# rwl/blu

Hardware: AMD Instinct MI355X
Metric: factorize nnz/s + achieved HBM GB/s, 100k x 100k 10-nnz/col basis (higher is better)
Workload: dtype f64

## Files before the change

### blu_amd/csrc/k_chain.h

```cpp
#pragma once
#include "blu_dev.h"

#define CH_SB 32
#define CH_NB 8
#define CH_CS (CH_SB * CH_NB)
#define CH_CE 4096
#define CH_W 2048
#define CH_FAR 320
#define CH_HAS 0x10000
#define CH_HT 16
#define CH_SEL_FAR (-1)
#define CH_SEL_PREV (-2)
#define CH_R 4
#define CH_TG 64
#define CH_SPIN 64

struct __attribute__((aligned(16))) ChRecA {
    int n, eb, w, k;
};
struct __attribute__((aligned(16))) ChRecB {
    double diag, own;
};
struct __attribute__((aligned(16))) ChOpsV {
    double val, xv;
};
struct ChainLds {
    ChOpsV ev[CH_CE];
    int sel[CH_CE];
    double xwin[CH_W];
    ChRecA ra[CH_CS];
    ChRecB rb[CH_CS];
    double rinit[CH_CS];
    long long s_b[CH_CS];
    volatile int blk_ready[CH_NB];
    volatile int eb_tag[CH_HT];
    volatile int eb_val[CH_HT];
    volatile int tag[CH_TG];
    volatile int ring_done[CH_R];
    volatile int ring_eb[CH_R];
    volatile int abort;
};

struct ChMeta {
    long long b;
    int len;
    int w;
    double diag, own;
};
struct ChEnt {
    int pos;
    int gidx;
    double val;
};

#ifdef BLU_EMU_BUILD
#define CH_LDS(T) T *
#else
#define CH_LDS(T) __attribute__((address_space(3))) T *
#endif
__device__ __forceinline__ int ch_flag(const volatile int *p) { return *(CH_LDS(const volatile int))p; }
__device__ __forceinline__ void ch_set(volatile int *p, int v) { *(CH_LDS(volatile int))p = v; }

#define CH_WAIT_SPIN(L, cond, code, spin, gave_up)                  \
    do {                                                            \
        int it_ = 0;                                                \
        while (!(cond)) {                                           \
            if (++it_ <= (spin)) continue;                          \
            if (ch_flag(&(L)->abort) || it_ > (1 << 24)) {                    \
                if (!ch_flag(&(L)->abort)) ch_set(&(L)->abort, (code));               \
                (gave_up) = true;                                   \
                break;                                              \
            }                                                       \
            __builtin_amdgcn_s_sleep(1);                            \
        }                                                           \
    } while (0)
#define CH_WAIT(L, cond, code)                       \
    do {                                             \
        bool gu_ = false;                            \
        CH_WAIT_SPIN(L, cond, code, 0, gu_);         \
    } while (0)

#ifdef BLU_EMU_BUILD
__device__ __forceinline__ void ch_lds_fence() {}
__device__ __forceinline__ void ch_vm_drain() {}
#else
__device__ __forceinline__ void ch_lds_fence() { asm volatile("s_waitcnt lgkmcnt(0)" ::: "memory"); }
__device__ __forceinline__ void ch_vm_drain() { asm volatile("s_waitcnt vmcnt(0)" ::: "memory"); }
#endif
__device__ __forceinline__ double ch_load_final(gdouble_p p)
{
    const long long b = __hip_atomic_load((GPTR(const long long))p, __ATOMIC_RELAXED, __HIP_MEMORY_SCOPE_AGENT);
    return __longlong_as_double(b);
}

__device__ __forceinline__ bool ch_room(ChainLds *L, int b, int top)
{
    int done = ch_flag(&L->ring_done[0]), eb = ch_flag(&L->ring_eb[0]);
#pragma unroll
    for (int r = 1; r < CH_R; r++) {
        const int d = ch_flag(&L->ring_done[r]), e = ch_flag(&L->ring_eb[r]);
        done = d < done ? d : done;
        eb = e < eb ? e : eb;
    }
    return done >= b - CH_NB + 1 && top - eb <= CH_CE;
}
template <bool INIT_OWN, bool SUB, class A>
__device__ __forceinline__ void ch_stage_block(const A &ad, ChainLds *L, int b, int k0, int dir, int nsteps, gdouble_p out)
{
    const int lane = lane_id();
    const int s0 = b * CH_SB;
    const int ns = nsteps - s0 < CH_SB ? nsteps - s0 : CH_SB;
    const int k = k0 + dir * (s0 + (lane < ns ? lane : 0));
    ChMeta M = ad.meta(k);
    if (M.len < 0) M.len = 0;
    const bool mine = lane < ns;
    const int st = (mine && M.len <= 64) ? M.len : 0;
    const int incl = wave_incl_scan_i(st);
    const int off = incl - st;
    const int cnt = __builtin_amdgcn_readlane(incl, 63);
    int base = 0;
    if (b > 0) {
        CH_WAIT(L, ch_flag(&L->eb_tag[b & (CH_HT - 1)]) == b, 1);
        base = ch_flag(&L->eb_val[b & (CH_HT - 1)]);
    }
    if (lane == 0) {
        ch_set(&L->eb_val[(b + 1) & (CH_HT - 1)], base + cnt);
        ch_lds_fence();
        ch_set(&L->eb_tag[(b + 1) & (CH_HT - 1)], b + 1);
    }
    CH_WAIT(L, ch_room(L, b, base + cnt), 2);
    asm volatile("" ::: "memory");
    if (ch_flag(&L->abort)) return;
    const int slot0 = s0 & (CH_CS - 1);
    if (mine) {
        const int sl = slot0 + lane;
        ChRecA a;
        a.n = M.len <= 64 ? (M.len > 0 ? (M.len | CH_HAS) : 0) : -1;
        a.eb = base + off;
        a.w = M.w;
        a.k = k;
        L->ra[sl] = a;
        ChRecB bq;
        bq.diag = M.diag;
        bq.own = M.own;
        L->rb[sl] = bq;
        L->rinit[sl] = INIT_OWN ? M.own : 0.0;
        L->s_b[sl] = M.b;
    }
    ch_lds_fence();
    for (int f0 = 0; f0 < cnt; f0 += 256) {
        int tt[4], ee[4];
        ChEnt E[4];
        bool ok[4], far[4];
        double xo[4];
#pragma unroll
        for (int u = 0; u < 4; u++) {
            const int f = f0 + u * 64 + lane;
            ok[u] = f < cnt;
            int lo = 0, hi = ns - 1;
            const int target = base + (ok[u] ? f : 0);
#pragma unroll
            for (int it = 0; it < 5; it++) {
                const int mid = (lo + hi + 1) >> 1;
                const bool ge = (L->ra[slot0 + mid].eb <= target) && (mid <= hi);
                lo = ge ? mid : lo;
                hi = ge ? hi : mid - 1;
            }
            tt[u] = lo;
            ee[u] = target - L->ra[slot0 + lo].eb;
        }
#pragma unroll
        for (int u = 0; u < 4; u++) {
            E[u].pos = 0;
            E[u].gidx = 0;
            E[u].val = 0.0;
            if (ok[u]) E[u] = ad.ent(L->ra[slot0 + tt[u]].k, L->s_b[slot0 + tt[u]], ee[u]);
        }
#pragma unroll
        for (int u = 0; u < 4; u++) {
            const int kk = L->ra[slot0 + tt[u]].k;
            const int d = (kk - E[u].pos) * dir;
            far[u] = ok[u] && d >= CH_FAR;
            xo[u] = 0.0;
            if (far[u]) xo[u] = ch_load_final(out + E[u].gidx);
        }
#pragma unroll
        for (int u = 0; u < 4; u++) {
            if (ok[u]) {
                const int kk = L->ra[slot0 + tt[u]].k;
                const int r = (base + f0 + u * 64 + lane) & (CH_CE - 1);
                ChOpsV ov;
                ov.val = E[u].val;
                ov.xv = xo[u];
                L->ev[r] = ov;
                L->sel[r] = far[u] ? CH_SEL_FAR : (E[u].pos == kk - dir ? CH_SEL_PREV : (E[u].pos & (CH_W - 1)));
            }
        }
    }
    ch_lds_fence();
    if (mine && M.len > 0 && M.len <= 64) {
        const int sl = slot0 + lane;
        const int eb = base + off;
        double acc = INIT_OWN ? M.own : 0.0;
        int p = 0;
        while (p < M.len && L->sel[(eb + p) & (CH_CE - 1)] == CH_SEL_FAR) {
            const ChOpsV ov = L->ev[(eb + p) & (CH_CE - 1)];
            const double term = __dmul_rn(ov.xv, ov.val);
            acc = SUB ? __dsub_rn(acc, term) : __dadd_rn(acc, term);
            p++;
        }
        if (p > 0) {
            L->ra[sl].n = (M.len - p) | CH_HAS;
            L->ra[sl].eb = eb + p;
            L->rinit[sl] = acc;
        }
    }
    ch_lds_fence();
    if (lane == 0) ch_set(&L->blk_ready[b & (CH_NB - 1)], b + 1);
}

struct ChRec {
    int n, eb, w, k;
    double diag, own, init;
};
struct ChOps {
    double val, xv;
    int sel;
};
__device__ __forceinline__ ChRec ch_read_rec(ChainLds *L, int s)
{
    const int sl = s & (CH_CS - 1);
    const ChRecA a = L->ra[sl];
    const ChRecB b = L->rb[sl];
    ChRec R;
    R.n = a.n;
    R.eb = a.eb;
    R.w = a.w;
    R.k = a.k;
    R.diag = b.diag;
    R.own = b.own;
    R.init = L->rinit[sl];
    return R;
}
template <bool SUB>
__device__ __forceinline__ double ch_accumulate(double acc, double prod, int n)
{
    const unsigned lo = (unsigned)__double_as_longlong(prod), hi = (unsigned)(__double_as_longlong(prod) >> 32);
#define CH_TERM(T)                                                                                              \
    {                                                                                                           \
        const unsigned a_ = __builtin_amdgcn_readlane(lo, (T)), b_ = __builtin_amdgcn_readlane(hi, (T));        \
        const double term_ = __longlong_as_double((long long)(((unsigned long long)b_ << 32) | a_));            \
        acc = SUB ? __dsub_rn(acc, term_) : __dadd_rn(acc, term_);                                              \
    }
    int t = 0;
    for (; t + 4 <= n; t += 4) {
        CH_TERM(t)
        CH_TERM(t + 1)
        CH_TERM(t + 2)
        CH_TERM(t + 3)
    }
    for (; t < n; t++) CH_TERM(t)
#undef CH_TERM
    return acc;
}

template <bool SUB>
__device__ __forceinline__ double ch_accumulate_rows(double acc, double prod, int n)
{
    const double sg = SUB ? -1.0 : 1.0;
#ifdef BLU_EMU_BUILD
#define CH_D(T) acc = fma(__shfl(prod, (lane_id() & ~15) + T), sg, acc);
#define CH_D0 CH_D(0)
#else
#define CH_D(T) asm volatile("v_fmac_f64_dpp %0, %1, %2 row_newbcast:" #T " row_mask:0xf bank_mask:0xf" : "+v"(acc) : "v"(prod), "v"(sg));
#define CH_D0 asm volatile("s_nop 4\n\tv_fmac_f64_dpp %0, %1, %2 row_newbcast:0 row_mask:0xf bank_mask:0xf" : "+v"(acc) : "v"(prod), "v"(sg));
#endif
#define CH_TAIL(A, B, C) \
    if (n > A) {         \
        CH_D(A)          \
        if (n > B) {     \
            CH_D(B)      \
            if (n > C) { \
                CH_D(C)  \
            }            \
        }                \
    }
    if (n >= 4) {
        CH_D0 CH_D(1) CH_D(2) CH_D(3)
        if (n >= 8) {
            CH_D(4) CH_D(5) CH_D(6) CH_D(7)
            if (n >= 12) {
                CH_D(8) CH_D(9) CH_D(10) CH_D(11)
                if (n >= 16) {
                    CH_D(12) CH_D(13) CH_D(14) CH_D(15)
                } else {
                    CH_TAIL(12, 13, 14)
                }
            } else {
                CH_TAIL(8, 9, 10)
            }
        } else {
            CH_TAIL(4, 5, 6)
        }
    } else if (n > 0) {
        CH_D0
        CH_TAIL(1, 2, 3)
    }
#undef CH_TAIL
#undef CH_D0
#undef CH_D
    return acc;
}

template <bool INIT_OWN, bool SUB, class A, class F>
__device__ __forceinline__ bool chain_sweep(const A &ad, ChainLds *L, int k0, int dir, int nsteps, gdouble_p out, F f)
{
    static_assert(CH_R >= 1 && CH_R <= CH_SB && CH_TG >= 2 * CH_R, "ring size");
    const int w = wave_id(), nw = num_waves(), lane = lane_id();
    const int nblk = (nsteps + CH_SB - 1) / CH_SB;
    if (threadIdx.x < CH_NB) ch_set(&L->blk_ready[threadIdx.x], 0);
    if (threadIdx.x < CH_HT) ch_set(&L->eb_tag[threadIdx.x], -1);
    if (threadIdx.x < CH_TG) ch_set(&L->tag[threadIdx.x], 0);
    if (threadIdx.x < CH_R) {
        ch_set(&L->ring_done[threadIdx.x], 0);
        ch_set(&L->ring_eb[threadIdx.x], 0);
    }
    if (threadIdx.x == 0) ch_set(&L->abort, 0);
    __syncthreads();
    if (w >= CH_R) {
        for (int b = w - CH_R; b < nblk && !ch_flag(&L->abort); b += nw - CH_R) ch_stage_block<INIT_OWN, SUB>(ad, L, b, k0, dir, nsteps, out);
    } else {
#ifdef BLU_PROFILE
        long long t_wait = 0, t_tag = 0, t_drain = 0;
        const long long t_begin = (long long)__builtin_amdgcn_s_memtime();
#endif
        const int last = nsteps - 1;
        const int li = lane & 15;
        __builtin_amdgcn_s_setprio(3);
        const auto rl_d = [](double x, int t) {
            const int lo = __builtin_amdgcn_readlane(__double2loint(x), t), hi = __builtin_amdgcn_readlane(__double2hiint(x), t);
            return __hiloint2double(hi, lo);
        };
        const auto read_ops = [&](int eb, int n) {
            ChOps E;
            E.val = 0.0;
            E.xv = 0.0;
            E.sel = CH_SEL_FAR;
            const int l = n <= 16 ? li : lane;
            if (l < n) {
                const int r = (eb + l) & (CH_CE - 1);
                const ChOpsV v = L->ev[r];
                E.val = v.val;
                E.xv = v.xv;
                E.sel = L->sel[r];
            }
            return E;
        };
        int cur_b = -1;
        ChRec BR;
        BR.n = BR.eb = BR.w = BR.k = 0;
        BR.diag = BR.own = BR.init = 0.0;
        bool gave_up = false;
        for (int s = w; s < nsteps && !gave_up; s += CH_R) {
            const int b = s / CH_SB;
            if (b != cur_b) {
                if (cur_b >= 0) {
#ifdef BLU_PROFILE
                    const long long td0 = (long long)__builtin_amdgcn_s_memtime();
#endif
                    ch_vm_drain();
#ifdef BLU_PROFILE
                    t_drain += (long long)__builtin_amdgcn_s_memtime() - td0;
#endif
                    ch_lds_fence();
                    if (lane == 0) ch_set(&L->ring_done[w], b);
                }
#ifdef BLU_PROFILE
                const long long tw0 = (long long)__builtin_amdgcn_s_memtime();
#endif
                CH_WAIT_SPIN(L, ch_flag(&L->blk_ready[b & (CH_NB - 1)]) == b + 1, 3, 0, gave_up);
                asm volatile("" ::: "memory");
#ifdef BLU_PROFILE
                t_wait += (long long)__builtin_amdgcn_s_memtime() - tw0;
#endif
                if (gave_up) break;
                const int sl = b * CH_SB + lane;
                BR = ch_read_rec(L, sl < last ? sl : last);
                if (lane == 0) ch_set(&L->ring_eb[w], BR.eb);
                cur_b = b;
            }
            const int t = s - b * CH_SB;
            const int nf = __builtin_amdgcn_readlane(BR.n, t), eb1 = __builtin_amdgcn_readlane(BR.eb, t);
            const int k1 = __builtin_amdgcn_readlane(BR.k, t), w1 = __builtin_amdgcn_readlane(BR.w, t);
            const double own1 = rl_d(BR.own, t), diag1 = rl_d(BR.diag, t);
            const int n1 = nf < 0 ? -1 : (nf & (CH_HAS - 1));
            double acc = rl_d(BR.init, t);
            const auto wait_prev = [&]() {
                if (s > 0) {
#ifdef BLU_PROFILE
                    const long long tw0 = (long long)__builtin_amdgcn_s_memtime();
#endif
                    CH_WAIT_SPIN(L, ch_flag(&L->tag[(s - 1) & (CH_TG - 1)]) == s, 4, CH_SPIN, gave_up);
#ifdef BLU_PROFILE
                    t_tag += (long long)__builtin_amdgcn_s_memtime() - tw0;
#endif
                }
                asm volatile("" ::: "memory");
            };
            const auto slot_of = [&](int sel) { return (sel == CH_SEL_PREV ? k1 - dir : sel) & (CH_W - 1); };
            const auto dist_of = [&](int slot) { return ((k1 - slot) * dir) & (CH_W - 1); };
            if (n1 > 0 && n1 <= 16) {
                const ChOps E = read_ops(eb1, n1);
                const int slot = slot_of(E.sel);
                const bool win = E.sel != CH_SEL_FAR;
                const bool late = win && dist_of(slot) < CH_R;
                const unsigned lm = (unsigned)__ballot(late) & 0xffffu;
                const int p = lm ? __ffs((int)lm) - 1 : n1;
                if (p > 0) {
                    const double x = (win && !late) ? L->xwin[slot] : E.xv;
                    acc = ch_accumulate_rows<SUB>(acc, li < p ? __dmul_rn(x, E.val) : 0.0, p);
                }
                if (p < n1) {
                    const int nl = n1 - p;
                    const ChOps EL = read_ops(eb1 + p, nl);
                    const int slot_l = slot_of(EL.sel);
                    const bool win_l = EL.sel != CH_SEL_FAR;
                    const bool late_l = win_l && dist_of(slot_l) < CH_R;
                    const double prod_e = __dmul_rn((win_l && !late_l) ? L->xwin[slot_l] : EL.xv, EL.val);
                    wait_prev();
                    const double prod_l = __dmul_rn(L->xwin[slot_l], EL.val);
                    acc = ch_accumulate_rows<SUB>(acc, li < nl ? (late_l ? prod_l : prod_e) : 0.0, nl);
                } else {
                    wait_prev();
                }
            } else if (n1 > 16) {
                const ChOps E = read_ops(eb1, n1);
                wait_prev();
                const double x = E.sel != CH_SEL_FAR ? L->xwin[slot_of(E.sel)] : E.xv;
                acc = ch_accumulate<SUB>(acc, lane < n1 ? __dmul_rn(x, E.val) : 0.0, n1);
            } else if (n1 < 0) {
                wait_prev();
                const ChMeta M = ad.meta(k1);
                for (int o = 0; o < M.len; o += 64) {
                    ChEnt E;
                    E.pos = k1 - dir * CH_FAR;
                    E.gidx = 0;
                    E.val = 0.0;
                    const int nn = M.len - o < 64 ? M.len - o : 64;
                    double x = 0.0;
                    if (lane < nn) {
                        E = ad.ent(k1, M.b, o + lane);
                        const int d = (k1 - E.pos) * dir;
                        x = (d > 0 && d < CH_FAR) ? L->xwin[E.pos & (CH_W - 1)] : ch_load_final(out + E.gidx);
                    }
                    acc = ch_accumulate<SUB>(acc, lane < nn ? __dmul_rn(x, E.val) : 0.0, nn);
                }
            } else {
                wait_prev();
            }
            if (gave_up) break;
            const double v = f(k1, nf != 0, acc, own1, diag1);
            if (lane == 0) {
                L->xwin[k1 & (CH_W - 1)] = v;
                ch_lds_fence();
                ch_set(&L->tag[s & (CH_TG - 1)], s + 1);
                out[w1] = v;
            }
        }
        __builtin_amdgcn_s_setprio(0);
        ch_vm_drain();
        ch_lds_fence();
        if (lane == 0) {
            ch_set(&L->ring_eb[w], 0x7fffffff);
            ch_set(&L->ring_done[w], nblk + CH_NB);
        }
#ifdef BLU_PROFILE
        if (lane == 0 && nsteps > 0)
            printf("chain sweep (block %d, ring wave %d of %d): %d steps, %.0f cycles/step of the sweep, waiting for blocks %.0f, for the predecessor %.0f, draining stores %.0f\n",
                   (int)blockIdx.x, w, CH_R, nsteps, (double)((long long)__builtin_amdgcn_s_memtime() - t_begin) / nsteps, (double)t_wait / nsteps,
                   (double)t_tag / nsteps, (double)t_drain / nsteps);
#endif
    }
    __syncthreads();
    return ch_flag(&L->abort) == 0;
}

__device__ __forceinline__ double ch_abs_sum_ordered(gdouble_p v, int k0, int dir, int n, double *vmax)
{
    const int lane = lane_id();
    const auto ld = [&](int s0) {
        const int s = s0 + lane;
        return s < n ? fabs(ch_load_final(v + (k0 + dir * s))) : 0.0;
    };
    double acc = 0.0, mx = 0.0;
    double a0 = ld(0), a1 = ld(64), a2 = ld(128), a3 = ld(192);
    for (int s0 = 0; s0 < n; s0 += 64) {
        const double cur = a0;
        a0 = a1;
        a1 = a2;
        a2 = a3;
        a3 = ld(s0 + 256);
        mx = fmax(mx, cur);
        const int nn = n - s0 < 64 ? n - s0 : 64;
        for (int c = 0; c < nn; c += 16) {
            const double rowv = __shfl(cur, c + (lane & 15));
            acc = ch_accumulate_rows<false>(acc, rowv, nn - c < 16 ? nn - c : 16);
        }
    }
    *vmax = wave_max_d(mx);
    return acc;
}
```

### blu_amd/csrc/k_chain.hip

```cpp
#include "blu_dev.h"
#include "k_chain.h"

struct RowsWs {
    int *lt_ptr, *lt_idx;
    double *lt_val;
    int *lt_cur;
    int *ur_len;
    int *ur_pos;
    double *ur_val;
};

template <bool DESC>
__device__ __forceinline__ void insertion_sort_ik(int *key, double *val, int b, int e)
{
    for (int p = b + 1; p < e; p++) {
        const int k = key[p];
        const double v = val[p];
        int q = p - 1;
        while (q >= b && (DESC ? key[q] < k : key[q] > k)) {
            key[q + 1] = key[q];
            val[q + 1] = val[q];
            q--;
        }
        key[q + 1] = k;
        val[q + 1] = v;
    }
}
template <bool DESC>
__device__ void wave_sort_segment_ik(int *key, double *val, int b, int e, int *lk, double *lv)
{
    const int lane = lane_id();
    const int n = e - b;
    WAVE_LOCKSTEP();
    for (int t = lane; t < n; t += 64) {
        lk[t] = key[b + t];
        lv[t] = val[b + t];
    }
    __builtin_amdgcn_fence(__ATOMIC_SEQ_CST, "workgroup");
    for (int t = lane; t < n; t += 64) {
        const int k = lk[t];
        int r = 0;
        for (int u = 0; u < n; u++) r += DESC ? (lk[u] > k) : (lk[u] < k);
        key[b + r] = k;
        val[b + r] = lv[t];
    }
}

template <class Scope>
__device__ __forceinline__ void rows_body(const DevG &D, const RowsWs &R, Scope &sc, int *lds_k, double *lds_v)
{
    Scalars *S = D.s;
    const int tid = sc.tid(), nt = sc.nt();
    const int m = D.m;
    if (S->status != ST_DONE) return;
    const int rank = S->rank;
    const int lend = D.lbeg[rank];
    for (int i = tid; i < m; i += nt) R.lt_cur[i] = 0;
    if (sc.leader()) *sc.ctr(0) = *sc.ctr(1) = 0;
    sc.sync();
    for (int p = tid; p < lend; p += nt) atomicAdd(&R.lt_cur[D.lidx[p]], 1);
    sc.sync();
    int base = 0;
    for (int c0 = 0; c0 < m; c0 += nt) {
        const int i = c0 + tid;
        const int c = i < m ? R.lt_cur[i] : 0;
        int tot;
        const int ex = sc.excl_scan(c, &tot);
        if (i < m) {
            R.lt_ptr[i] = base + ex;
            R.lt_cur[i] = base + ex;
        }
        base += tot;
    }
    if (sc.leader()) R.lt_ptr[m] = base;
    sc.sync();
    for (int k = tid; k < rank; k += nt)
        for (int p = D.lbeg[k]; p < D.lbeg[k + 1]; p++) {
            const int q = atomicAdd(&R.lt_cur[D.lidx[p]], 1);
            R.lt_idx[q] = k;
            R.lt_val[q] = D.lval[p];
        }
    sc.sync();
    for (int i = tid; i < m; i += nt) {
        const int b = R.lt_ptr[i], e = R.lt_ptr[i + 1];
        if (e - b > 24 && e - b <= WSORT_MAX) D.iw2[atomicAdd(sc.ctr(0), 1)] = i;
        else insertion_sort_ik<false>(R.lt_idx, R.lt_val, b, e);
    }
    for (int k = tid; k < m; k += nt) {
        int n = 0;
        if (k < rank) {
            const int b = D.ubeg[k], e = D.ubeg[k + 1];
            for (int p = b; p < e; p++) {
                const int c = D.qinv[D.uidx[p]];
                if (c < rank) {
                    R.ur_pos[b + n] = c;
                    R.ur_val[b + n] = D.uval[p];
                    n++;
                }
            }
            if (n > 24 && n <= WSORT_MAX) D.iw1[atomicAdd(sc.ctr(1), 1)] = k;
            else insertion_sort_ik<true>(R.ur_pos, R.ur_val, b, b + n);
        }
        R.ur_len[k] = n;
    }
    sc.sync();
    {
        const int nl = __hip_atomic_load(sc.ctr(0), __ATOMIC_RELAXED, __HIP_MEMORY_SCOPE_AGENT);
        const int nu = __hip_atomic_load(sc.ctr(1), __ATOMIC_RELAXED, __HIP_MEMORY_SCOPE_AGENT);
#ifdef BLU_STATS_DEBUG
        if (sc.leader()) printf("k_rows_grid: medium L rows %d, medium U rows %d, rank %d, m %d\n", nl, nu, rank, m);
#endif
        for (int r = sc.wid(); r < nl + nu; r += sc.nw()) {
            if (r < nl) {
                const int i = D.iw2[r];
                wave_sort_segment_ik<false>(R.lt_idx, R.lt_val, R.lt_ptr[i], R.lt_ptr[i + 1], &lds_k[wave_id() * WSORT_MAX],
                                            &lds_v[wave_id() * WSORT_MAX]);
            } else {
                const int k = D.iw1[r - nl];
                wave_sort_segment_ik<true>(R.ur_pos, R.ur_val, D.ubeg[k], D.ubeg[k] + R.ur_len[k], &lds_k[wave_id() * WSORT_MAX],
                                           &lds_v[wave_id() * WSORT_MAX]);
            }
        }
    }
    sc.sync();
    for (int p = tid; p < lend; p += nt) R.lt_idx[p] = D.prow[R.lt_idx[p]];
}
__global__ void __launch_bounds__(1024) k_rows_grid(DevLU *Ds, GridWs *gw, RowsWs R)
{
    __shared__ int sh[40];
    __shared__ long long shl[20];
    __shared__ int lds_k[16 * WSORT_MAX];
    __shared__ double lds_v[16 * WSORT_MAX];
    const DevG D(Ds[0]);
    GridScope sc{sh, shl, gw, 0};
    rows_body(D, R, sc, lds_k, lds_v);
}

struct ChUCols {
    GPTR(const long long) colptr;
    GPTR(const long long) rowidx;
    GPTR(const double) value;
    gdouble_p own;
    __device__ __forceinline__ ChMeta meta(int k) const
    {
        ChMeta M;
        M.b = colptr[k];
        const long long e = colptr[k + 1] - 1;
        M.len = (int)(e - M.b);
        M.w = k;
        M.diag = value[e];
        M.own = own ? ch_load_final(own + k) : 0.0;
        return M;
    }
    __device__ __forceinline__ ChEnt ent(int, long long b, int e) const
    {
        ChEnt E;
        E.pos = (int)rowidx[b + e];
        E.gidx = E.pos;
        E.val = value[b + e];
        return E;
    }
};
struct ChLStage {
    gcint_p lbeg, lidx, pinv;
    gdouble_p lval;
    gdouble_p own;
    __device__ __forceinline__ ChMeta meta(int k) const
    {
        ChMeta M;
        M.b = lbeg[k];
        M.len = lbeg[k + 1] - lbeg[k];
        M.w = k;
        M.diag = 1.0;
        M.own = own ? ch_load_final(own + k) : 0.0;
        return M;
    }
    __device__ __forceinline__ ChEnt ent(int, long long b, int e) const
    {
        ChEnt E;
        E.pos = pinv[lidx[b + e]];
        E.gidx = E.pos;
        E.val = lval[b + e];
        return E;
    }
};
struct ChLRows {
    const int *ptr, *idx;
    const double *v;
    gcint_p prow, pinv;
    gdouble_p own;
    __device__ __forceinline__ ChMeta meta(int k) const
    {
        ChMeta M;
        const int i = prow[k];
        M.b = ptr[i];
        M.len = ptr[i + 1] - ptr[i];
        M.w = k;
        M.diag = 1.0;
        M.own = own ? ch_load_final(own + k) : 0.0;
        return M;
    }
    __device__ __forceinline__ ChEnt ent(int, long long b, int e) const
    {
        ChEnt E;
        E.pos = pinv[idx[b + e]];
        E.gidx = E.pos;
        E.val = v[b + e];
        return E;
    }
};
struct ChURows {
    gcint_p ubeg;
    const int *len, *pos;
    const double *v;
    GPTR(const long long) colptr;
    GPTR(const double) value;
    gdouble_p own;
    __device__ __forceinline__ ChMeta meta(int k) const
    {
        ChMeta M;
        M.b = ubeg[k];
        M.len = len[k];
        M.w = k;
        M.diag = value[colptr[k + 1] - 1];
        M.own = own ? ch_load_final(own + k) : 0.0;
        return M;
    }
    __device__ __forceinline__ ChEnt ent(int, long long b, int e) const
    {
        ChEnt E;
        E.pos = pos[b + e];
        E.gidx = E.pos;
        E.val = v[b + e];
        return E;
    }
};

#define CHAIN_THREADS 512
static_assert(CHAIN_THREADS / 64 > CH_R, "the chain kernels need at least one helper wave");
__global__ void __launch_bounds__(CHAIN_THREADS) k_stats_chains(DevLU *Ds, FinishOut *Os, RowsWs R, int *defect)
{
    BLU_DYN_SHARED(unsigned char, ch_smem, sizeof(ChainLds));
    ChainLds *L = (ChainLds *)ch_smem;
    const DevG D(Ds[0]);
    const FinishOut &O = Os[0];
    Scalars *S = D.s;
    const int m = D.m, lane = lane_id();
    if (S->status != ST_DONE || D.skip_stats) return;
    const size_t M1 = (size_t)(m + 1);
    gdouble_p wl = D.gwork, wu = D.gwork + M1, lf = D.gwork + 2 * M1, rf = D.gwork + 3 * M1, lb = D.gwork + 4 * M1, rb = D.gwork + 5 * M1;
    gdouble_p res = D.gwork + 8 * M1;
    const bool w0 = threadIdx.x < 64;
    const int cc = blockIdx.x;
    bool ok = true;
    const auto abs_sum = [&](gdouble_p v, int k0, int dir, double *vmax) {
#ifdef BLU_PROFILE
        const long long t0 = (long long)__builtin_amdgcn_s_memtime();
#endif
        const double sum = ch_abs_sum_ordered(v, k0, dir, m, vmax);
#ifdef BLU_PROFILE
        if (lane == 0)
            printf("ordered sum of |x| (block %d): %d terms, %.1f cycles/term\n", (int)blockIdx.x, m, (double)((long long)__builtin_amdgcn_s_memtime() - t0) / (m > 0 ? m : 1));
#endif
        return sum;
    };
    if (cc == 0) {
        double x1 = 0.0, xinf = 0.0, y1 = 0.0, ymax;
        const ChLStage A1{D.lbeg, D.lidx, D.pinv, D.lval, nullptr};
        ok = ok && chain_sweep<false, false>(A1, L, m - 1, -1, m, wl, [&](int, bool has, double dot, double, double) {
            double temp = has ? -dot : 0.0;
            temp += temp >= 0.0 ? 1.0 : -1.0;
            return temp;
        });
        if (w0 && ok) x1 = abs_sum(wl, m - 1, -1, &xinf);
        const ChLRows A2{R.lt_ptr, R.lt_idx, R.lt_val, D.prow, D.pinv, wl};
        ok = ok && chain_sweep<true, true>(A2, L, 0, 1, m, wl, [&](int, bool, double acc, double, double) { return acc; });
        if (w0 && ok) y1 = abs_sum(wl, 0, 1, &ymax);
        if (w0 && lane == 0) res[0] = fmax(y1 / x1, xinf);
    } else if (cc == 1) {
        double x1 = 0.0, xinf = 0.0, y1 = 0.0, ymax;
        const ChUCols A1{(GPTR(const long long))O.u_colptr, (GPTR(const long long))O.u_rowidx, (GPTR(const double))O.u_value, nullptr};
        ok = ok && chain_sweep<false, false>(A1, L, 0, 1, m, wu, [&](int, bool has, double dot, double, double diag) {
            double temp = has ? -dot : 0.0;
            temp += temp >= 0.0 ? 1.0 : -1.0;
            temp /= diag;
            return temp;
        });
        if (w0 && ok) x1 = abs_sum(wu, 0, 1, &xinf);
        const ChURows A2{D.ubeg, R.ur_len, R.ur_pos, R.ur_val, (GPTR(const long long))O.u_colptr, (GPTR(const double))O.u_value, wu};
        ok = ok && chain_sweep<true, true>(A2, L, m - 1, -1, m, wu, [&](int, bool, double acc, double, double diag) { return acc / diag; });
        if (w0 && ok) y1 = abs_sum(wu, m - 1, -1, &ymax);
        if (w0 && lane == 0) res[1] = fmax(y1 / x1, xinf);
    } else if (cc == 2) {
        const ChLRows A1{R.lt_ptr, R.lt_idx, R.lt_val, D.prow, D.pinv, nullptr};
        ok = ok && chain_sweep<false, false>(A1, L, 0, 1, m, lf, [&](int k, bool, double d, double, double) {
            const double r = d <= 0.0 ? 1.0 : -1.0;
            if (lane == 0) rf[k] = r;
            return r - d;
        });
        const ChURows A2{D.ubeg, R.ur_len, R.ur_pos, R.ur_val, (GPTR(const long long))O.u_colptr, (GPTR(const double))O.u_value, lf};
        ok = ok && chain_sweep<true, true>(A2, L, m - 1, -1, m, lf, [&](int, bool, double acc, double, double diag) { return acc / diag; });
    } else {
        const ChUCols A1{(GPTR(const long long))O.u_colptr, (GPTR(const long long))O.u_rowidx, (GPTR(const double))O.u_value, nullptr};
        ok = ok && chain_sweep<false, false>(A1, L, 0, 1, m, lb, [&](int k, bool has, double dot, double, double diag) {
            const double d = has ? dot : 0.0;
            const double r = d <= 0.0 ? 1.0 : -1.0;
            if (lane == 0) rb[k] = r;
            return (r - d) / diag;
        });
        const ChLStage A2{D.lbeg, D.lidx, D.pinv, D.lval, lb};
        ok = ok && chain_sweep<false, false>(A2, L, m - 1, -1, m, lb, [&](int, bool has, double dot, double own, double) { return has ? own - dot : own; });
    }
    if (!ok && threadIdx.x == 0) atomicMax(defect, ch_flag(&L->abort) ? ch_flag(&L->abort) : 99);
}

#define TAIL_BLOCKS 64
__global__ void __launch_bounds__(1024) k_stats_tail_a(DevLU *Ds, FinishOut *Os, GridWs *gw)
{
    const DevG D(Ds[0]);
    const FinishOut &O = Os[0];
    Scalars *S = D.s;
    __shared__ double red[4][40];
    if (S->status != ST_DONE || D.skip_stats) return;
    double v[4];
    stats_tail_loops<false>(D, O, (int)(blockIdx.x * blockDim.x + threadIdx.x), (int)(gridDim.x * blockDim.x), v[0], v[1], v[2], v[3],
                            &gw->nlong);
    for (int q = 0; q < 4; q++) {
        const double x = wave_max_d(v[q]);
        if (lane_id() == 0) red[q][wave_id()] = x;
    }
    __syncthreads();
    if (threadIdx.x < 4) {
        double a = red[threadIdx.x][0];
        for (int ww = 1; ww < num_waves(); ww++) a = fmax(a, red[threadIdx.x][ww]);
        ((double *)gw->partll[0])[4 * blockIdx.x + threadIdx.x] = a;
    }
}
__global__ void __launch_bounds__(1024) k_stats_tail_b(DevLU *Ds, FinishOut *Os, GridWs *gw)
{
    const DevG D(Ds[0]);
    Scalars *S = D.s;
    __shared__ double red[4][40];
    __shared__ double chain_out[16];
    if (S->status != ST_DONE || D.skip_stats) return;
    const size_t M1 = (size_t)(D.m + 1);
    if (threadIdx.x < 2) chain_out[threadIdx.x] = D.gwork[8 * M1 + threadIdx.x];
    double v[4] = {0.0, 0.0, 0.0, 0.0};
    if (threadIdx.x < TAIL_BLOCKS)
        for (int q = 0; q < 4; q++) v[q] = ((const double *)gw->partll[0])[4 * threadIdx.x + q];
    const int nlong = gw->nlong;
    if (nlong && wave_id() < 4)
        v[3] = fmax(v[3], stats_long_rows(D.bt_ptr, D.bt_idx, D.bt_val, D.qinv, D.pinv, D.gwork, D.m, S->rank, nlong, wave_id(), 4));
    __syncthreads();
    stats_tail_finish(D, red, chain_out, v[0], v[1], v[2], v[3]);
    if (threadIdx.x < 2) D.gwork[8 * M1 + threadIdx.x] = 0.0;
}

struct ChSolveLRows {
    const int *ptr, *idx;
    const double *v;
    gcint_p prow, pinv;
    gdouble_p y;
    __device__ __forceinline__ ChMeta meta(int k) const
    {
        ChMeta M;
        const int i = prow[k];
        M.b = ptr[i];
        M.len = ptr[i + 1] - ptr[i];
        M.w = i;
        M.diag = 1.0;
        M.own = ch_load_final(y + i);
        return M;
    }
    __device__ __forceinline__ ChEnt ent(int, long long b, int e) const
    {
        ChEnt E;
        E.gidx = idx[b + e];
        E.pos = pinv[E.gidx];
        E.val = v[b + e];
        return E;
    }
};
struct ChSolveURows {
    gcint_p ubeg;
    const int *len, *pos;
    const double *v;
    GPTR(const long long) colptr;
    GPTR(const double) value;
    gcint_p prow, pcol;
    gdouble_p y;
    __device__ __forceinline__ ChMeta meta(int k) const
    {
        ChMeta M;
        M.b = ubeg[k];
        M.len = len[k];
        M.w = pcol[k];
        M.diag = value[colptr[k + 1] - 1];
        M.own = ch_load_final(y + prow[k]);
        return M;
    }
    __device__ __forceinline__ ChEnt ent(int, long long b, int e) const
    {
        ChEnt E;
        E.pos = pos[b + e];
        E.gidx = pcol[E.pos];
        E.val = v[b + e];
        return E;
    }
};
struct ChSolveUCols {
    GPTR(const long long) colptr;
    GPTR(const long long) rowidx;
    GPTR(const double) value;
    gcint_p prow, pcol;
    gdouble_p y;
    __device__ __forceinline__ ChMeta meta(int k) const
    {
        ChMeta M;
        M.b = colptr[k];
        const long long e = colptr[k + 1] - 1;
        M.len = (int)(e - M.b);
        M.w = prow[k];
        M.diag = value[e];
        M.own = ch_load_final(y + pcol[k]);
        return M;
    }
    __device__ __forceinline__ ChEnt ent(int, long long b, int e) const
    {
        ChEnt E;
        E.pos = (int)rowidx[b + e];
        E.gidx = prow[E.pos];
        E.val = value[b + e];
        return E;
    }
};
struct ChSolveLStage {
    gcint_p lbeg, lidx, pinv, prow;
    gdouble_p lval;
    gdouble_p x;
    __device__ __forceinline__ ChMeta meta(int k) const
    {
        ChMeta M;
        M.b = lbeg[k];
        M.len = lbeg[k + 1] - lbeg[k];
        M.w = prow[k];
        M.diag = 1.0;
        M.own = ch_load_final(x + M.w);
        return M;
    }
    __device__ __forceinline__ ChEnt ent(int, long long b, int e) const
    {
        ChEnt E;
        E.gidx = lidx[b + e];
        E.pos = pinv[E.gidx];
        E.val = lval[b + e];
        return E;
    }
};

__global__ void __launch_bounds__(CHAIN_THREADS) k_solve_dense_chain(DevLU *Ds, FinishOut *Os, RowsWs R, const double *rhs, double *lhs, int trans,
                                                                     int *defect)
{
    BLU_DYN_SHARED(unsigned char, ch_smem, sizeof(ChainLds));
    ChainLds *L = (ChainLds *)ch_smem;
    const DevG D(Ds[0]);
    const FinishOut &O = Os[0];
    const int m = D.m;
    gdouble_p y = D.txrj;
    gdouble_p x_out = (gdouble_p)lhs;
    for (int k = threadIdx.x; k < m; k += blockDim.x) y[k] = rhs[k];
    ch_vm_drain();
    __syncthreads();
    const auto sub_dot = [](int, bool has, double dot, double own, double) { return has ? own - dot : own; };
    const auto over_diag = [](int, bool, double acc, double, double diag) { return acc / diag; };
    bool ok = true;
    if (!trans) {
        const ChSolveLRows A1{R.lt_ptr, R.lt_idx, R.lt_val, D.prow, D.pinv, y};
        ok = ok && chain_sweep<false, false>(A1, L, 0, 1, m, y, sub_dot);
        const ChSolveURows A2{D.ubeg, R.ur_len, R.ur_pos, R.ur_val, (GPTR(const long long))O.u_colptr, (GPTR(const double))O.u_value, D.prow, D.pcol, y};
        ok = ok && chain_sweep<true, true>(A2, L, m - 1, -1, m, x_out, over_diag);
    } else {
        const ChSolveUCols A1{(GPTR(const long long))O.u_colptr, (GPTR(const long long))O.u_rowidx, (GPTR(const double))O.u_value, D.prow, D.pcol, y};
        ok = ok && chain_sweep<true, true>(A1, L, 0, 1, m, x_out, over_diag);
        const ChSolveLStage A2{D.lbeg, D.lidx, D.pinv, D.prow, D.lval, x_out};
        ok = ok && chain_sweep<false, false>(A2, L, m - 1, -1, m, x_out, sub_dot);
    }
    if (threadIdx.x == 0) *defect = ok ? 0 : 9100 + ch_flag(&L->abort);
}
```

Baseline: 1.546 million.

## Publish chain values with tags in a single LDS vector write

Swaps the separate xwin store, LDS fence and tag flag for a 16-byte record that carries the value halves, each tagged with its step, written in one vector store. Consumers poll the record itself and take the value straight from it, and late terms wait only on the specific predecessor slot they need instead of always on the immediately previous step. This removes the lgkmcnt fence and a dependent LDS reload from the serial step-to-step hand-over. It relies on the 128-bit LDS write being seen as a unit (checked through both tag copies) and adds a DIV template parameter plus profiling counters.

```diff
diff --git a/blu_amd/csrc/k_chain.h b/blu_amd/csrc/k_chain.h
--- a/blu_amd/csrc/k_chain.h
+++ b/blu_amd/csrc/k_chain.h
@@ -24,6 +24,10 @@
 struct __attribute__((aligned(16))) ChOpsV {
     double val, xv;
 };
+struct __attribute__((aligned(16))) ChPub {
+    unsigned lo, tag_lo, hi, tag_hi;
+};
+typedef unsigned ch_u4 __attribute__((ext_vector_type(4)));
 struct ChainLds {
     ChOpsV ev[CH_CE];
     int sel[CH_CE];
@@ -35,7 +39,7 @@
     volatile int blk_ready[CH_NB];
     volatile int eb_tag[CH_HT];
     volatile int eb_val[CH_HT];
-    volatile int tag[CH_TG];
+    ChPub pub[CH_TG];
     volatile int ring_done[CH_R];
     volatile int ring_eb[CH_R];
     volatile int abort;
@@ -60,6 +64,17 @@
 #endif
 __device__ __forceinline__ int ch_flag(const volatile int *p) { return *(CH_LDS(const volatile int))p; }
 __device__ __forceinline__ void ch_set(volatile int *p, int v) { *(CH_LDS(volatile int))p = v; }
+
+__device__ __forceinline__ ch_u4 ch_pub_read(const ChPub *p) { return *(CH_LDS(const volatile ch_u4))p; }
+__device__ __forceinline__ void ch_pub_write(ChPub *p, double v, int tag)
+{
+    ch_u4 q;
+    q.x = (unsigned)__double2loint(v);
+    q.y = (unsigned)tag;
+    q.z = (unsigned)__double2hiint(v);
+    q.w = (unsigned)tag;
+    *(CH_LDS(volatile ch_u4))p = q;
+}
 
 #define CH_WAIT_SPIN(L, cond, code, spin, gave_up)                  \
     do {                                                            \
@@ -83,10 +98,13 @@
 #ifdef BLU_EMU_BUILD
 __device__ __forceinline__ void ch_lds_fence() {}
 __device__ __forceinline__ void ch_vm_drain() {}
+__device__ __forceinline__ void ch_pin(double &) {}
 #else
 __device__ __forceinline__ void ch_lds_fence() { asm volatile("s_waitcnt lgkmcnt(0)" ::: "memory"); }
 __device__ __forceinline__ void ch_vm_drain() { asm volatile("s_waitcnt vmcnt(0)" ::: "memory"); }
-#endif
+__device__ __forceinline__ void ch_pin(double &x) { asm volatile("" : "+v"(x)); }
+#endif
+
 __device__ __forceinline__ double ch_load_final(gdouble_p p)
 {
     const long long b = __hip_atomic_load((GPTR(const long long))p, __ATOMIC_RELAXED, __HIP_MEMORY_SCOPE_AGENT);
@@ -312,15 +330,15 @@
     return acc;
 }
 
-template <bool INIT_OWN, bool SUB, class A, class F>
+template <bool INIT_OWN, bool SUB, bool DIV, class A, class F>
 __device__ __forceinline__ bool chain_sweep(const A &ad, ChainLds *L, int k0, int dir, int nsteps, gdouble_p out, F f)
 {
     static_assert(CH_R >= 1 && CH_R <= CH_SB && CH_TG >= 2 * CH_R, "ring size");
-    const int w = wave_id(), nw = num_waves(), lane = lane_id();
+    const int w = __builtin_amdgcn_readfirstlane(wave_id()), nw = num_waves(), lane = lane_id();
     const int nblk = (nsteps + CH_SB - 1) / CH_SB;
     if (threadIdx.x < CH_NB) ch_set(&L->blk_ready[threadIdx.x], 0);
     if (threadIdx.x < CH_HT) ch_set(&L->eb_tag[threadIdx.x], -1);
-    if (threadIdx.x < CH_TG) ch_set(&L->tag[threadIdx.x], 0);
+    if (threadIdx.x < CH_TG) ch_pub_write(&L->pub[threadIdx.x], 0.0, 0);
     if (threadIdx.x < CH_R) {
         ch_set(&L->ring_done[threadIdx.x], 0);
         ch_set(&L->ring_eb[threadIdx.x], 0);
@@ -332,6 +350,8 @@
     } else {
 #ifdef BLU_PROFILE
         long long t_wait = 0, t_tag = 0, t_drain = 0;
+        long long ph_c[5] = {0, 0, 0, 0, 0}, t_seen = 0;
+        int ph_n[5] = {0, 0, 0, 0, 0};
         const long long t_begin = (long long)__builtin_amdgcn_s_memtime();
 #endif
         const int last = nsteps - 1;
@@ -395,17 +415,38 @@
             const double own1 = rl_d(BR.own, t), diag1 = rl_d(BR.diag, t);
             const int n1 = nf < 0 ? -1 : (nf & (CH_HAS - 1));
             double acc = rl_d(BR.init, t);
+#ifdef BLU_PROFILE
+            int kind = n1 < 0 ? 4 : (n1 > 16 ? 3 : 0);
+#endif
+            const auto wait_slots = [&](int d, double &x) {
+                ch_pin(acc);
+                if (s > 0) {
+#ifdef BLU_PROFILE
+                    const long long tw0 = (long long)__builtin_amdgcn_s_memtime();
+#endif
+                    const int sp = s - d;
+                    const ChPub *slot = &L->pub[sp & (CH_TG - 1)];
+                    const unsigned want = (unsigned)(sp + 1);
+                    ch_u4 q = ch_pub_read(slot);
+                    bool have = __ballot(q.y != want || q.w != want) == 0;
+                    for (int it = 1; !have && it < CH_SPIN; it++) {
+                        q = ch_pub_read(slot);
+                        have = __ballot(q.y != want || q.w != want) == 0;
+                    }
+                    if (!have) CH_WAIT_SPIN(L, (q = ch_pub_read(slot), __ballot(q.y != want || q.w != want) == 0), 4, 0, gave_up);
+                    x = __hiloint2double((int)q.z, (int)q.x);
+#ifdef BLU_PROFILE
+                    t_tag += (long long)__builtin_amdgcn_s_memtime() - tw0;
+#endif
+                }
+#ifdef BLU_PROFILE
+                t_seen = (long long)__builtin_amdgcn_s_memtime();
+#endif
+                asm volatile("" ::: "memory");
+            };
             const auto wait_prev = [&]() {
-                if (s > 0) {
-#ifdef BLU_PROFILE
-                    const long long tw0 = (long long)__builtin_amdgcn_s_memtime();
-#endif
-                    CH_WAIT_SPIN(L, ch_flag(&L->tag[(s - 1) & (CH_TG - 1)]) == s, 4, CH_SPIN, gave_up);
-#ifdef BLU_PROFILE
-                    t_tag += (long long)__builtin_amdgcn_s_memtime() - tw0;
-#endif
-                }
-                asm volatile("" ::: "memory");
+                double x_unused = 0.0;
+                wait_slots(1, x_unused);
             };
             const auto slot_of = [&](int sel) { return (sel == CH_SEL_PREV ? k1 - dir : sel) & (CH_W - 1); };
             const auto dist_of = [&](int slot) { return ((k1 - slot) * dir) & (CH_W - 1); };
@@ -425,10 +466,15 @@
                     const ChOps EL = read_ops(eb1 + p, nl);
                     const int slot_l = slot_of(EL.sel);
                     const bool win_l = EL.sel != CH_SEL_FAR;
-                    const bool late_l = win_l && dist_of(slot_l) < CH_R;
+                    const int d_l = dist_of(slot_l);
+                    const bool late_l = win_l && d_l >= 1 && d_l < CH_R && d_l <= s;
                     const double prod_e = __dmul_rn((win_l && !late_l) ? L->xwin[slot_l] : EL.xv, EL.val);
-                    wait_prev();
-                    const double prod_l = __dmul_rn(L->xwin[slot_l], EL.val);
+#ifdef BLU_PROFILE
+                    kind = __popcll(__ballot(late_l && lane < nl)) >= 3 ? 2 : 1;
+#endif
+                    double x_l = 0.0;
+                    wait_slots((late_l && lane != 63) ? d_l : 1, x_l);
+                    const double prod_l = __dmul_rn(x_l, EL.val);
                     acc = ch_accumulate_rows<SUB>(acc, li < nl ? (late_l ? prod_l : prod_e) : 0.0, nl);
                 } else {
                     wait_prev();
@@ -462,10 +508,21 @@
             const double v = f(k1, nf != 0, acc, own1, diag1);
             if (lane == 0) {
                 L->xwin[k1 & (CH_W - 1)] = v;
-                ch_lds_fence();
-                ch_set(&L->tag[s & (CH_TG - 1)], s + 1);
+                asm volatile("" ::: "memory");
+                ch_pub_write(&L->pub[s & (CH_TG - 1)], v, s + 1);
                 out[w1] = v;
             }
+#ifdef BLU_PROFILE
+            {
+                const long long dt = (long long)__builtin_amdgcn_s_memtime() - t_seen;
+#pragma unroll
+                for (int q = 0; q < 5; q++)
+                    if (kind == q) {
+                        ph_c[q] += dt;
+                        ph_n[q]++;
+                    }
+            }
+#endif
         }
         __builtin_amdgcn_s_setprio(0);
         ch_vm_drain();
@@ -479,6 +536,12 @@
             printf("chain sweep (block %d, ring wave %d of %d): %d steps, %.0f cycles/step of the sweep, waiting for blocks %.0f, for the predecessor %.0f, draining stores %.0f\n",
                    (int)blockIdx.x, w, CH_R, nsteps, (double)((long long)__builtin_amdgcn_s_memtime() - t_begin) / nsteps, (double)t_wait / nsteps,
                    (double)t_tag / nsteps, (double)t_drain / nsteps);
+        if (lane == 0 && nsteps > 0) {
+            const auto per = [](long long c, int n) { return n ? (double)c / n : 0.0; };
+            printf("chain hand-over (block %d, ring wave %d, division %d): cycles from tag seen to tag written, per step [steps]: no late term %.0f [%d] | 1-2 late terms %.0f [%d] | 3+ late terms %.0f [%d] | 17-64 entries %.0f [%d] | long %.0f [%d]\n",
+                   (int)blockIdx.x, w, (int)DIV, per(ph_c[0], ph_n[0]), ph_n[0], per(ph_c[1], ph_n[1]), ph_n[1], per(ph_c[2], ph_n[2]), ph_n[2],
+                   per(ph_c[3], ph_n[3]), ph_n[3], per(ph_c[4], ph_n[4]), ph_n[4]);
+        }
 #endif
     }
     __syncthreads();
diff --git a/blu_amd/csrc/k_chain.hip b/blu_amd/csrc/k_chain.hip
--- a/blu_amd/csrc/k_chain.hip
+++ b/blu_amd/csrc/k_chain.hip
@@ -267,20 +267,20 @@
     if (cc == 0) {
         double x1 = 0.0, xinf = 0.0, y1 = 0.0, ymax;
         const ChLStage A1{D.lbeg, D.lidx, D.pinv, D.lval, nullptr};
-        ok = ok && chain_sweep<false, false>(A1, L, m - 1, -1, m, wl, [&](int, bool has, double dot, double, double) {
+        ok = ok && chain_sweep<false, false, false>(A1, L, m - 1, -1, m, wl, [&](int, bool has, double dot, double, double) {
             double temp = has ? -dot : 0.0;
             temp += temp >= 0.0 ? 1.0 : -1.0;
             return temp;
         });
         if (w0 && ok) x1 = abs_sum(wl, m - 1, -1, &xinf);
         const ChLRows A2{R.lt_ptr, R.lt_idx, R.lt_val, D.prow, D.pinv, wl};
-        ok = ok && chain_sweep<true, true>(A2, L, 0, 1, m, wl, [&](int, bool, double acc, double, double) { return acc; });
+        ok = ok && chain_sweep<true, true, false>(A2, L, 0, 1, m, wl, [&](int, bool, double acc, double, double) { return acc; });
         if (w0 && ok) y1 = abs_sum(wl, 0, 1, &ymax);
         if (w0 && lane == 0) res[0] = fmax(y1 / x1, xinf);
     } else if (cc == 1) {
         double x1 = 0.0, xinf = 0.0, y1 = 0.0, ymax;
         const ChUCols A1{(GPTR(const long long))O.u_colptr, (GPTR(const long long))O.u_rowidx, (GPTR(const double))O.u_value, nullptr};
-        ok = ok && chain_sweep<false, false>(A1, L, 0, 1, m, wu, [&](int, bool has, double dot, double, double diag) {
+        ok = ok && chain_sweep<false, false, true>(A1, L, 0, 1, m, wu, [&](int, bool has, double dot, double, double diag) {
             double temp = has ? -dot : 0.0;
             temp += temp >= 0.0 ? 1.0 : -1.0;
             temp /= diag;
@@ -288,28 +288,28 @@
         });
         if (w0 && ok) x1 = abs_sum(wu, 0, 1, &xinf);
         const ChURows A2{D.ubeg, R.ur_len, R.ur_pos, R.ur_val, (GPTR(const long long))O.u_colptr, (GPTR(const double))O.u_value, wu};
-        ok = ok && chain_sweep<true, true>(A2, L, m - 1, -1, m, wu, [&](int, bool, double acc, double, double diag) { return acc / diag; });
+        ok = ok && chain_sweep<true, true, true>(A2, L, m - 1, -1, m, wu, [&](int, bool, double acc, double, double diag) { return acc / diag; });
         if (w0 && ok) y1 = abs_sum(wu, m - 1, -1, &ymax);
         if (w0 && lane == 0) res[1] = fmax(y1 / x1, xinf);
     } else if (cc == 2) {
         const ChLRows A1{R.lt_ptr, R.lt_idx, R.lt_val, D.prow, D.pinv, nullptr};
-        ok = ok && chain_sweep<false, false>(A1, L, 0, 1, m, lf, [&](int k, bool, double d, double, double) {
+        ok = ok && chain_sweep<false, false, false>(A1, L, 0, 1, m, lf, [&](int k, bool, double d, double, double) {
             const double r = d <= 0.0 ? 1.0 : -1.0;
             if (lane == 0) rf[k] = r;
             return r - d;
         });
         const ChURows A2{D.ubeg, R.ur_len, R.ur_pos, R.ur_val, (GPTR(const long long))O.u_colptr, (GPTR(const double))O.u_value, lf};
-        ok = ok && chain_sweep<true, true>(A2, L, m - 1, -1, m, lf, [&](int, bool, double acc, double, double diag) { return acc / diag; });
+        ok = ok && chain_sweep<true, true, true>(A2, L, m - 1, -1, m, lf, [&](int, bool, double acc, double, double diag) { return acc / diag; });
     } else {
         const ChUCols A1{(GPTR(const long long))O.u_colptr, (GPTR(const long long))O.u_rowidx, (GPTR(const double))O.u_value, nullptr};
-        ok = ok && chain_sweep<false, false>(A1, L, 0, 1, m, lb, [&](int k, bool has, double dot, double, double diag) {
+        ok = ok && chain_sweep<false, false, true>(A1, L, 0, 1, m, lb, [&](int k, bool has, double dot, double, double diag) {
             const double d = has ? dot : 0.0;
             const double r = d <= 0.0 ? 1.0 : -1.0;
             if (lane == 0) rb[k] = r;
             return (r - d) / diag;
         });
         const ChLStage A2{D.lbeg, D.lidx, D.pinv, D.lval, lb};
-        ok = ok && chain_sweep<false, false>(A2, L, m - 1, -1, m, lb, [&](int, bool has, double dot, double own, double) { return has ? own - dot : own; });
+        ok = ok && chain_sweep<false, false, false>(A2, L, m - 1, -1, m, lb, [&](int, bool has, double dot, double own, double) { return has ? own - dot : own; });
     }
     if (!ok && threadIdx.x == 0) atomicMax(defect, ch_flag(&L->abort) ? ch_flag(&L->abort) : 99);
 }
@@ -476,14 +476,14 @@
     bool ok = true;
     if (!trans) {
         const ChSolveLRows A1{R.lt_ptr, R.lt_idx, R.lt_val, D.prow, D.pinv, y};
-        ok = ok && chain_sweep<false, false>(A1, L, 0, 1, m, y, sub_dot);
+        ok = ok && chain_sweep<false, false, false>(A1, L, 0, 1, m, y, sub_dot);
         const ChSolveURows A2{D.ubeg, R.ur_len, R.ur_pos, R.ur_val, (GPTR(const long long))O.u_colptr, (GPTR(const double))O.u_value, D.prow, D.pcol, y};
-        ok = ok && chain_sweep<true, true>(A2, L, m - 1, -1, m, x_out, over_diag);
+        ok = ok && chain_sweep<true, true, true>(A2, L, m - 1, -1, m, x_out, over_diag);
     } else {
         const ChSolveUCols A1{(GPTR(const long long))O.u_colptr, (GPTR(const long long))O.u_rowidx, (GPTR(const double))O.u_value, D.prow, D.pcol, y};
-        ok = ok && chain_sweep<true, true>(A1, L, 0, 1, m, x_out, over_diag);
+        ok = ok && chain_sweep<true, true, true>(A1, L, 0, 1, m, x_out, over_diag);
         const ChSolveLStage A2{D.lbeg, D.lidx, D.pinv, D.prow, D.lval, x_out};
-        ok = ok && chain_sweep<false, false>(A2, L, m - 1, -1, m, x_out, sub_dot);
+        ok = ok && chain_sweep<false, false, false>(A2, L, m - 1, -1, m, x_out, sub_dot);
     }
     if (threadIdx.x == 0) *defect = ok ? 0 : 9100 + ch_flag(&L->abort);
 }
```

Result: no change. 1.558 million (median of 6 runs) (+0.8%).
